# psy-ex/svt-av1-psy

Hardware: AMD Instinct MI355X
Metric: Mblocks/s per kernel (SAD, FwdTxfm2d, CDEF) + encoder fps @1080p preset 8 (higher is better)
Workload: dtype u8

## Files before the change

### svt-av1-psy_amd/csrc/sad.hip

```cpp
#include "svt_hip_common.h"
#include "../../include/svtav1_hip.h"
#include "hme_geom.h"
#include <vector>

namespace {

struct __attribute__((packed, aligned(4))) U64A4 { unsigned long long v; };
struct __attribute__((aligned(4))) u32x4_a4 { uint32_t x, y, z, w; };
struct __attribute__((aligned(16))) u32x4_a16 { uint32_t x, y, z, w; };

constexpr uint32_t MAX_SAD_VALUE = 128 * 128 * 255;
constexpr int      ME_TW         = 64;
constexpr int      ME_TH         = 32;
constexpr int      KEY_POS_BITS  = 11;
constexpr uint32_t ME_WAVE_MAX_W = 24, ME_WAVE_MAX_H = 16;

__device__ __forceinline__ void stage_rows_u8(uint32_t* lds, int pitch_dw, const uint8_t* g, uint32_t gstride, int width,
                                              int rows, int tid, int nthreads) {
    const int total = rows * pitch_dw;
    for (int i = tid; i < total; i += nthreads) {
        const int r   = i / pitch_dw;
        const int k   = i - r * pitch_dw;
        const int col = k * 4;
        uint32_t  v   = 0;
        if (col < width) {
            const uint8_t*  p    = g + (size_t)r * gstride + col;
            const uint32_t  sh   = (uint32_t)((uintptr_t)p & 3);
            const uint32_t* ap   = (const uint32_t*)(p - sh);
            const int       need = (width - col) < 4 ? (width - col) : 4;
            const uint32_t  lo   = ap[0];
            uint32_t        hi   = 0;
            if ((int)sh + need > 4) hi = ap[1];
            v = __builtin_amdgcn_alignbyte(hi, lo, sh);
            if (need < 4) v &= (1u << (8 * need)) - 1u;
        }
        lds[i] = v;
    }
}

struct __attribute__((packed, aligned(1))) u32x4_a1 { uint32_t x, y, z, w; };
struct __attribute__((packed, aligned(1))) u32_a1 { uint32_t x; };
struct __attribute__((aligned(8))) u32x2_a8 { uint32_t x, y; };

template <int NIT, int CL2>
__device__ __forceinline__ void stage_rows_load(uint32_t (&v)[NIT][4], const uint8_t* g, uint32_t gstride, int width, int rows, int tid) {
#pragma unroll
    for (int k = 0; k < NIT; ++k) {
        const int  idx = tid + 256 * k, r = idx >> CL2, col = (idx & ((1 << CL2) - 1)) * 16;
        const bool live = r < rows && col < width;
        const int  left = width - col;
        const int  back = (live && left < 16) ? 16 - left : 0;
        const uint8_t* p = g + (live ? (size_t)r * gstride + (size_t)(col - back) : (size_t)0);
        const u32x4_a1 t = *(const u32x4_a1*)p;
        v[k][0] = t.x; v[k][1] = t.y; v[k][2] = t.z; v[k][3] = t.w;
    }
#pragma unroll
    for (int k = 0; k < NIT; ++k) {
        const int  idx = tid + 256 * k, r = idx >> CL2, col = (idx & ((1 << CL2) - 1)) * 16;
        const bool live = r < rows && col < width;
        const int  left = width - col;
        uint32_t   x0 = live ? v[k][0] : 0u, x1 = live ? v[k][1] : 0u, x2 = live ? v[k][2] : 0u, x3 = live ? v[k][3] : 0u;
        if (live && left < 16) {
            const int back = 16 - left;
            if (back & 4) { x0 = x1; x1 = x2; x2 = x3; x3 = 0; }
            if (back & 8) { x0 = x2; x1 = x3; x2 = 0; x3 = 0; }
            const uint32_t bs = (uint32_t)back & 3u;
            x0 = __builtin_amdgcn_alignbyte(x1, x0, bs);
            x1 = __builtin_amdgcn_alignbyte(x2, x1, bs);
            x2 = __builtin_amdgcn_alignbyte(x3, x2, bs);
            x3 = __builtin_amdgcn_alignbyte(0u, x3, bs);
        }
        v[k][0] = x0; v[k][1] = x1; v[k][2] = x2; v[k][3] = x3;
    }
}
template <int NIT, int CL2>
__device__ __forceinline__ void stage_rows_store(const uint32_t (&v)[NIT][4], uint32_t* lds, int pitch_dw, int rows, int tid) {
#pragma unroll
    for (int k = 0; k < NIT; ++k) {
        const int idx = tid + 256 * k, r = idx >> CL2, c4 = (idx & ((1 << CL2) - 1)) * 4;
        if (r < rows) {
            uint32_t* o = lds + r * pitch_dw + c4;
            if (c4 + 0 < pitch_dw) *(u32x2_a8*)(o + 0) = u32x2_a8{v[k][0], v[k][1]};
            if (c4 + 2 < pitch_dw) *(u32x2_a8*)(o + 2) = u32x2_a8{v[k][2], v[k][3]};
        }
    }
}

template <int NT, int U>
__device__ __forceinline__ void stage_rows_wide_step(uint32_t* lds, const int pitch_dw, const uint8_t* g, const uint32_t gstride, const int width, const int total,
                                                     const int cpr, const int dr, const int dc, const int base, const int tid, int& r, int& c) {
    uint32_t v[U][4];
    int      rk[U], ck[U];
#pragma unroll
    for (int k = 0; k < U; ++k) {
        const int  idx = base + tid + NT * k, col = c * 16;
        rk[k] = r; ck[k] = c;
        const bool live = idx < total && col < width;
        const int  left = width - col;
        const int  back = (live && left < 16) ? 16 - left : 0;
        const uint8_t* p = g + (live ? (uint32_t)r * gstride + (uint32_t)(col - back) : 0u);
        const u32x4_a1 t = *(const u32x4_a1*)p;
        uint32_t x0 = live ? t.x : 0u, x1 = live ? t.y : 0u, x2 = live ? t.z : 0u, x3 = live ? t.w : 0u;
        if (back) {
            if (back & 4) { x0 = x1; x1 = x2; x2 = x3; x3 = 0; }
            if (back & 8) { x0 = x2; x1 = x3; x2 = 0; x3 = 0; }
            const uint32_t bs = (uint32_t)back & 3u;
            x0 = __builtin_amdgcn_alignbyte(x1, x0, bs);
            x1 = __builtin_amdgcn_alignbyte(x2, x1, bs);
            x2 = __builtin_amdgcn_alignbyte(x3, x2, bs);
            x3 = __builtin_amdgcn_alignbyte(0u, x3, bs);
        }
        v[k][0] = x0; v[k][1] = x1; v[k][2] = x2; v[k][3] = x3;
        r += dr; c += dc;
        if (c >= cpr) { c -= cpr; r++; }
    }
#pragma unroll
    for (int k = 0; k < U; ++k) {
        const int idx = base + tid + NT * k, c4 = ck[k] * 4;
        if (idx < total) {
            uint32_t* o = lds + rk[k] * pitch_dw + c4;
            if (c4 + 0 < pitch_dw) *(u32x2_a8*)(o + 0) = u32x2_a8{v[k][0], v[k][1]};
            if (c4 + 2 < pitch_dw) *(u32x2_a8*)(o + 2) = u32x2_a8{v[k][2], v[k][3]};
        }
    }
}
template <int NT = 256>
__device__ __forceinline__ void stage_rows_wide_any(uint32_t* lds, int pitch_dw, const uint8_t* g, uint32_t gstride, int width, int rows, int tid) {
    const int cpr = (pitch_dw + 3) >> 2, total = rows * cpr;
    const int dr = NT / cpr, dc = NT - dr * cpr;
    int       r = tid / cpr, c = tid - r * cpr;
    int base = 0;
    for (; total - base > 2 * NT; base += 4 * NT) stage_rows_wide_step<NT, 4>(lds, pitch_dw, g, gstride, width, total, cpr, dr, dc, base, tid, r, c);
    if (total - base > NT) stage_rows_wide_step<NT, 2>(lds, pitch_dw, g, gstride, width, total, cpr, dr, dc, base, tid, r, c);
    else if (total - base > 0) stage_rows_wide_step<NT, 1>(lds, pitch_dw, g, gstride, width, total, cpr, dr, dc, base, tid, r, c);
}

__device__ __forceinline__ uint32_t dpp_add_quad_xor1(uint32_t v) {
    return v + (uint32_t)__builtin_amdgcn_update_dpp(0, (int)v, 0xB1, 0xf, 0xf, false);
}
__device__ __forceinline__ uint32_t dpp_add_quad_xor2(uint32_t v) {
    return v + (uint32_t)__builtin_amdgcn_update_dpp(0, (int)v, 0x4E, 0xf, 0xf, false);
}
__device__ __forceinline__ uint32_t dpp_add_row_ror4(uint32_t v) {
    return v + (uint32_t)__builtin_amdgcn_update_dpp(0, (int)v, 0x124, 0xf, 0xf, false);
}
__device__ __forceinline__ uint32_t dpp_add_row_ror8(uint32_t v) {
    return v + (uint32_t)__builtin_amdgcn_update_dpp(0, (int)v, 0x128, 0xf, 0xf, false);
}
__device__ __forceinline__ uint32_t umin32(uint32_t a, uint32_t b) { return a < b ? a : b; }


constexpr int ME_PITCH = 34;

__device__ __forceinline__ uint32_t dpp_scatter_sum_quads(const uint32_t (&v)[4]) {
#ifdef SVT_HIP_EMU
    const uint32_t a0 = dpp_add_row_ror8(v[0]), a1 = dpp_add_row_ror8(v[1]), a2 = dpp_add_row_ror8(v[2]), a3 = dpp_add_row_ror8(v[3]);
    const uint32_t t0 = (uint32_t)__builtin_amdgcn_update_dpp((int)a0, (int)a2, 0xE4, 0xf, 0xc, false);
    const uint32_t t1 = (uint32_t)__builtin_amdgcn_update_dpp((int)a1, (int)a3, 0xE4, 0xf, 0xc, false);
    const uint32_t y  = (uint32_t)__builtin_amdgcn_update_dpp((int)t0, (int)t1, 0xE4, 0xf, 0xa, false);
    const uint32_t x  = y + (uint32_t)__builtin_amdgcn_update_dpp(0, (int)t0, 0x12C, 0xf, 0x5, false);
    return x + (uint32_t)__builtin_amdgcn_update_dpp(0, (int)t1, 0x124, 0xf, 0xa, false);
#else
    uint32_t t0, t1;
    asm("s_nop 1\n\t"
        "v_add_u32_dpp %0, %2, %2 row_ror:8 row_mask:0xf bank_mask:0x3\n\t"
        "v_add_u32_dpp %0, %4, %4 row_ror:8 row_mask:0xf bank_mask:0xc\n\t"
        "v_add_u32_dpp %1, %3, %3 row_ror:8 row_mask:0xf bank_mask:0x3\n\t"
        "v_add_u32_dpp %1, %5, %5 row_ror:8 row_mask:0xf bank_mask:0xc\n\t"
        "v_add_u32_dpp %0, %0, %0 row_ror:12 row_mask:0xf bank_mask:0x5\n\t"
        "s_nop 0\n\t"
        "v_add_u32_dpp %0, %1, %1 row_ror:4 row_mask:0xf bank_mask:0xa"
        : "=&v"(t0), "=&v"(t1)
        : "v"(v[0]), "v"(v[1]), "v"(v[2]), "v"(v[3]));
    return t0;
#endif
}

template <bool SUB, bool FULL, int PITCH = ME_PITCH>
__device__ __forceinline__ void me_search_strips(const uint32_t* __restrict__ win, const uint32_t (&s)[8][2], int Wt, int Ht, int g0, int gstep, int l,
                                                 uint32_t& best8, uint32_t& best16, uint32_t& best32, uint32_t& best64) {
    const int bx = (l & 1) | ((l >> 1) & 2) | ((l >> 2) & 4);
    const int by = ((l >> 1) & 1) | ((l >> 2) & 2) | ((l >> 3) & 4);
    const int q  = l & 3, c = (l >> 2) & 3;
    const int      G    = (Wt + 3) >> 2;
    const uint32_t qsel = 0x0c0c0100u + 0x0202u * (uint32_t)q;
    uint32_t       himask = 0xffff0000u;
    SVT_HIP_OPAQUE_I32(himask);
    constexpr uint32_t NO_STEP = 0x1ffffu;
    uint32_t       b16 = 0xffffffffu, b32 = 0xffffffffu, b64 = 0xffffffffu;
    for (int g = g0; g < G; g += gstep) {
        const uint32_t* colp   = win + (by * 8) * PITCH + bx * 2 + g;
        const int       nvalid = (Wt - 4 * g) < 4 ? (Wt - 4 * g) : 4;
        const uint32_t inv1 = nvalid > 1 ? 0u : 0xffffffffu, inv2 = nvalid > 2 ? 0u : 0xffffffffu, inv3 = nvalid > 3 ? 0u : 0xffffffffu;
        const uint32_t invq = q < nvalid ? 0u : 0xffffffffu;
        U64A4 ra[8], rb[8];
#pragma unroll
        for (int r = 0; r < 7; r++) {
            ra[r] = *(const U64A4*)(colp + r * PITCH);
            rb[r] = *(const U64A4*)(colp + r * PITCH + 1);
        }
        uint32_t pos = (uint32_t)(4 * g);
        for (int yb = 0; yb < Ht; yb += 8) {
            const uint32_t* rowp = colp + (yb + 7) * PITCH;
#pragma unroll
            for (int h = 0; h < 2; h++) {
                if (yb + 4 * h < Ht) {
                    uint32_t v[4] = {NO_STEP, NO_STEP, NO_STEP, NO_STEP};
#pragma unroll
                    for (int j = 0; j < 4; j++) {
                        const int i = 4 * h + j;
                        if (yb + i < Ht) {
                            ra[(i + 7) & 7] = *(const U64A4*)(rowp + i * PITCH);
                            rb[(i + 7) & 7] = *(const U64A4*)(rowp + i * PITCH + 1);
                            unsigned long long acc = 0;
#pragma unroll
                            for (int r = 0; r < 8; r += (SUB ? 2 : 1)) {
                                acc = __builtin_amdgcn_qsad_pk_u16_u8(ra[(i + r) & 7].v, s[r][0], acc);
                                acc = __builtin_amdgcn_qsad_pk_u16_u8(rb[(i + r) & 7].v, s[r][1], acc);
                            }
                            if (SUB) acc <<= 1;
                            const uint32_t lo = (uint32_t)acc, hi = (uint32_t)(acc >> 32);
                            const uint32_t p1 = FULL ? pos + 1 : ((pos + 1) | inv1), p2 = FULL ? pos + 2 : ((pos + 2) | inv2), p3 = FULL ? pos + 3 : ((pos + 3) | inv3);
                            const uint32_t k0 = (lo << 16) | pos, k1 = (lo & himask) | p1, k2 = (hi << 16) | p2, k3 = (hi & himask) | p3;
                            best8 = umin32(umin32(best8, k0), k1);
                            best8 = umin32(umin32(best8, k2), k3);
                            const uint32_t tlo = dpp_add_quad_xor2(dpp_add_quad_xor1(lo));
                            const uint32_t thi = dpp_add_quad_xor2(dpp_add_quad_xor1(hi));
                            v[j] = __builtin_amdgcn_perm(thi, tlo, qsel);
                            const uint32_t k16 = (v[j] << KEY_POS_BITS) | pos;
                            b16 = umin32(b16, FULL ? k16 : (k16 | invq));
                            pos += ME_TW;
                        }
                    }
                    const uint32_t gpos  = (uint32_t)(4 * g + ME_TW * (yb + 4 * h));
                    const uint32_t sad32 = dpp_scatter_sum_quads(v);
                    const uint32_t k32   = (sad32 << KEY_POS_BITS) | gpos;
                    b32 = umin32(b32, FULL ? k32 : (k32 | invq));
                    const auto     x16   = __builtin_amdgcn_permlane16_swap(sad32, sad32, false, false);
                    const uint32_t pair  = x16[0] + x16[1];
                    const auto     x32   = __builtin_amdgcn_permlane32_swap(pair, pair, false, false);
                    const uint32_t sad64 = x32[0] + x32[1];
                    const uint32_t k64   = (sad64 << KEY_POS_BITS) | gpos;
                    b64 = umin32(b64, FULL ? k64 : (k64 | invq));
                }
            }
        }
    }
    best16 = umin32(best16, b16 | (uint32_t)q);
    best32 = umin32(best32, b32 | (uint32_t)(q | (c << 6)));
    best64 = umin32(best64, b64 | (uint32_t)(q | (c << 6)));
}

template <bool SUB>
__global__ __launch_bounds__(256, 4) void me_fullpel_kernel(const uint8_t* __restrict__ src_base, const uint8_t* __restrict__ ref_base,
                                                         const SvtHipMeSearchDesc* __restrict__ descs, uint32_t n,
                                                         uint32_t tiles_x,
                                                         uint32_t* __restrict__ best_sad, uint32_t* __restrict__ best_mv,
                                                         unsigned long long* __restrict__ keys) {
    HIP_DYNAMIC_SHARED(uint32_t, smem)
    uint32_t* src_lds  = smem;
    uint32_t* best_lds = smem + 64 * 16;
    uint32_t* win      = smem + 64 * 16 + 88;

    const int      tid  = threadIdx.x;
    const uint32_t item = xcd_remap(blockIdx.x, n);
    const uint32_t tile = blockIdx.y;
    const SvtHipMeSearchDesc d = descs[item];
    const int W   = d.search_area_width, H = d.search_area_height;
    const int tx0 = (int)(tile % tiles_x) * ME_TW;
    const int ty0 = (int)(tile / tiles_x) * ME_TH;
    if (tx0 >= W || ty0 >= H) {
        if (tile == 0 && keys == nullptr && tid < SVT_HIP_ME_NUM_BLOCKS) {
            best_sad[(size_t)item * SVT_HIP_ME_NUM_BLOCKS + tid] = MAX_SAD_VALUE;
            best_mv[(size_t)item * SVT_HIP_ME_NUM_BLOCKS + tid]  = 0;
        }
        return;
    }
    const int Wt = (W - tx0) < ME_TW ? (W - tx0) : ME_TW;
    const int Ht = (H - ty0) < ME_TH ? (H - ty0) : ME_TH;

    {
        uint32_t vs[1][4], vw[3][4];
        stage_rows_load<1, 2>(vs, src_base + d.src_off, d.src_stride, 64, 64, tid);
        stage_rows_load<3, 3>(vw, ref_base + d.ref_off + (size_t)ty0 * d.ref_stride + tx0, d.ref_stride, 64 + Wt - 1, 64 + Ht - 1, tid);
        stage_rows_store<1, 2>(vs, src_lds, 16, 64, tid);
        stage_rows_store<3, 3>(vw, win, ME_PITCH, 64 + Ht - 1, tid);
    }
    if (tid < 88) best_lds[tid] = 0xffffffffu;
    __syncthreads();

    const int l  = tid & 63;
    const int wv = tid >> 6;
    uint32_t s[8][2];
    {
        const int bx = (l & 1) | ((l >> 1) & 2) | ((l >> 2) & 4);
        const int by = ((l >> 1) & 1) | ((l >> 2) & 2) | ((l >> 3) & 4);
#pragma unroll
        for (int r = 0; r < 8; r++) {
            s[r][0] = src_lds[(by * 8 + r) * 16 + bx * 2 + 0];
            s[r][1] = src_lds[(by * 8 + r) * 16 + bx * 2 + 1];
        }
    }
    uint32_t best8 = 0xffffffffu, best16 = 0xffffffffu, best32 = 0xffffffffu, best64 = 0xffffffffu;
    if ((Wt & 3) == 0) me_search_strips<SUB, true>(win, s, Wt, Ht, wv, 4, l, best8, best16, best32, best64);
    else me_search_strips<SUB, false>(win, s, Wt, Ht, wv, 4, l, best8, best16, best32, best64);

    atomicMin(&best_lds[21 + l], best8);
    atomicMin(&best_lds[5 + (l >> 2)], best16);
    atomicMin(&best_lds[1 + (l >> 4)], best32);
    atomicMin(&best_lds[0], best64);
    __syncthreads();
    if (tid < SVT_HIP_ME_NUM_BLOCKS) {
        const uint32_t key = best_lds[tid];
        const uint32_t sad = tid >= 21 ? (key >> 16) : (key >> KEY_POS_BITS);
        const int      X   = tx0 + (int)(key & 63u);
        const int      Y   = ty0 + (int)((key >> 6) & 31u);
        const size_t   o   = (size_t)item * SVT_HIP_ME_NUM_BLOCKS + tid;
        if (keys == nullptr) {
            best_sad[o] = sad;
            best_mv[o]  = ((uint32_t)(uint16_t)(Y + d.y_search_area_origin) << 16) | (uint16_t)(X + d.x_search_area_origin);
        } else {
            atomicMin(&keys[o], ((unsigned long long)sad << 32) | (unsigned long long)(uint32_t)(Y * W + X));
        }
    }
}

struct __attribute__((packed, aligned(1))) u32x2_a1 { uint32_t x, y; };
__device__ __forceinline__ uint32_t dpp_min_quad_xor1(uint32_t v) { return umin32(v, (uint32_t)__builtin_amdgcn_update_dpp(-1, (int)v, 0xB1, 0xf, 0xf, false)); }
__device__ __forceinline__ uint32_t dpp_min_quad_xor2(uint32_t v) { return umin32(v, (uint32_t)__builtin_amdgcn_update_dpp(-1, (int)v, 0x4E, 0xf, 0xf, false)); }
__device__ __forceinline__ uint32_t dpp_min_row_ror4(uint32_t v) { return umin32(v, (uint32_t)__builtin_amdgcn_update_dpp(-1, (int)v, 0x124, 0xf, 0xf, false)); }
__device__ __forceinline__ uint32_t dpp_min_row_ror8(uint32_t v) { return umin32(v, (uint32_t)__builtin_amdgcn_update_dpp(-1, (int)v, 0x128, 0xf, 0xf, false)); }

template <int NF, int PITCH>
__device__ __forceinline__ void stage_window_wave(uint32_t* lds, const uint8_t* g, const uint32_t gstride, const int width, const int rows, const int l) {
    constexpr int RPI = 64 / NF;
    const int     rem = width & 15, back = 16 - rem;
    const bool    p0 = rem != 0 && l < rows, p1 = rem != 0 && l + 64 < rows;
    u32x4_a1      t[2] = {{0u, 0u, 0u, 0u}, {0u, 0u, 0u, 0u}};
    const uint32_t tail_off = (uint32_t)l * gstride + (uint32_t)(width - 16);
    if (p0) t[0] = *(const u32x4_a1*)(g + tail_off);
    if (p1) t[1] = *(const u32x4_a1*)(g + (size_t)64 * gstride + tail_off);

    const int lr = l / NF, lc = l - lr * NF;
    if (lr < RPI) {
        const uint32_t goff = (uint32_t)lr * gstride + (uint32_t)lc * 16u;
        uint32_t*      lp   = lds + lr * PITCH + lc * 4;
        for (int r0 = 0; r0 < rows; r0 += 4 * RPI) {
            const uint8_t* gb = g + (size_t)r0 * gstride;
            u32x4_a1       v[4];
#pragma unroll
            for (int k = 0; k < 4; k++)
                if (r0 + k * RPI + lr < rows) v[k] = *(const u32x4_a1*)(gb + (size_t)(k * RPI) * gstride + goff);
#pragma unroll
            for (int k = 0; k < 4; k++)
                if (r0 + k * RPI + lr < rows) {
                    uint32_t* o = lp + (r0 + k * RPI) * PITCH;
                    *(u32x2_a8*)(o + 0) = u32x2_a8{v[k].x, v[k].y};
                    *(u32x2_a8*)(o + 2) = u32x2_a8{v[k].z, v[k].w};
                }
        }
    }
#pragma unroll
    for (int k = 0; k < 2; k++)
        if (k == 0 ? p0 : p1) {
            uint32_t x0 = t[k].x, x1 = t[k].y, x2 = t[k].z, x3 = t[k].w;
            if (back & 4) { x0 = x1; x1 = x2; x2 = x3; x3 = 0; }
            if (back & 8) { x0 = x2; x1 = x3; x2 = 0; x3 = 0; }
            const uint32_t bs = (uint32_t)back & 3u;
            x0 = __builtin_amdgcn_alignbyte(x1, x0, bs);
            x1 = __builtin_amdgcn_alignbyte(x2, x1, bs);
            x2 = __builtin_amdgcn_alignbyte(x3, x2, bs);
            x3 = __builtin_amdgcn_alignbyte(0u, x3, bs);
            uint32_t* o = lds + (l + 64 * k) * PITCH + NF * 4;
            if (NF * 4 + 0 < PITCH) *(u32x2_a8*)(o + 0) = u32x2_a8{x0, x1};
            if (NF * 4 + 2 < PITCH) *(u32x2_a8*)(o + 2) = u32x2_a8{x2, x3};
        }
}

template <bool SUB, int PITCH>
__global__ __launch_bounds__(256) void me_fullpel_wave_kernel(const uint8_t* __restrict__ src_base, const uint8_t* __restrict__ ref_base,
                                                              const SvtHipMeSearchDesc* __restrict__ descs, const uint32_t n, const int win_dw,
                                                              uint32_t* __restrict__ best_sad, uint32_t* __restrict__ best_mv) {
    HIP_DYNAMIC_SHARED(uint32_t, smem)
    const int      l    = threadIdx.x & 63, wv = __builtin_amdgcn_readfirstlane((int)(threadIdx.x >> 6));
    const uint32_t item = xcd_remap(blockIdx.x, gridDim.x) * 4 + (uint32_t)wv;
    if (item >= n) return;
    const SvtHipMeSearchDesc d = descs[item];
    const int    W = d.search_area_width, H = d.search_area_height;
    const size_t o = (size_t)item * SVT_HIP_ME_NUM_BLOCKS;
    if (W <= 0 || H <= 0) {
        for (int k = l; k < SVT_HIP_ME_NUM_BLOCKS; k += 64) { best_sad[o + k] = MAX_SAD_VALUE; best_mv[o + k] = 0; }
        return;
    }
    uint32_t* win = smem + wv * win_dw;
    const int bx = (l & 1) | ((l >> 1) & 2) | ((l >> 2) & 4);
    const int by = ((l >> 1) & 1) | ((l >> 2) & 2) | ((l >> 3) & 4);
    uint32_t  s[8][2];
    {
        const uint8_t* sp = src_base + d.src_off + (size_t)(by * 8) * d.src_stride + bx * 8;
#pragma unroll
        for (int r = 0; r < 8; r++) {
            const u32x2_a1 t = *(const u32x2_a1*)(sp + (size_t)r * d.src_stride);
            s[r][0] = t.x; s[r][1] = t.y;
        }
    }
    const int width = 64 + W - 1;
    if (PITCH >= 22 && (width >> 4) == 5) stage_window_wave<5, PITCH>(win, ref_base + d.ref_off, d.ref_stride, width, 64 + H - 1, l);
    else stage_window_wave<4, PITCH>(win, ref_base + d.ref_off, d.ref_stride, width, 64 + H - 1, l);
    __builtin_amdgcn_wave_barrier();

    uint32_t best8 = 0xffffffffu, best16 = 0xffffffffu, best32 = 0xffffffffu, best64 = 0xffffffffu;
    if ((W & 3) == 0) me_search_strips<SUB, true, PITCH>(win, s, W, H, 0, 1, l, best8, best16, best32, best64);
    else me_search_strips<SUB, false, PITCH>(win, s, W, H, 0, 1, l, best8, best16, best32, best64);
    best16 = dpp_min_quad_xor2(dpp_min_quad_xor1(best16));
    best32 = dpp_min_row_ror8(dpp_min_row_ror4(dpp_min_quad_xor2(dpp_min_quad_xor1(best32))));
    best64 = dpp_min_row_ror8(dpp_min_row_ror4(dpp_min_quad_xor2(dpp_min_quad_xor1(best64))));
    best64 = umin32(best64, (uint32_t)__shfl_xor((int)best64, 16));
    best64 = umin32(best64, (uint32_t)__shfl_xor((int)best64, 32));
    const int xo = d.x_search_area_origin, yo = d.y_search_area_origin;
    auto emit = [&](const int idx, const uint32_t key, const bool is8) {
        const uint32_t sad = is8 ? (key >> 16) : (key >> KEY_POS_BITS);
        const int      X = (int)(key & 63u), Y = (int)((key >> 6) & 31u);
        best_sad[o + idx] = sad;
        best_mv[o + idx]  = ((uint32_t)(uint16_t)(Y + yo) << 16) | (uint16_t)(X + xo);
    };
    emit(21 + l, best8, true);
    if ((l & 3) == 0) emit(5 + (l >> 2), best16, false);
    if ((l & 15) == 0) emit(1 + (l >> 4), best32, false);
    if (l == 0) emit(0, best64, false);
}

__global__ void me_finalize_kernel(const SvtHipMeSearchDesc* __restrict__ descs, uint32_t n, const unsigned long long* __restrict__ keys,
                                   uint32_t* __restrict__ best_sad, uint32_t* __restrict__ best_mv) {
    const uint32_t i = blockIdx.x * blockDim.x + threadIdx.x;
    if (i >= n * SVT_HIP_ME_NUM_BLOCKS) return;
    const SvtHipMeSearchDesc d   = descs[i / SVT_HIP_ME_NUM_BLOCKS];
    const unsigned long long key = keys[i];
    if (key == ~0ull) {
        best_sad[i] = MAX_SAD_VALUE;
        best_mv[i]  = 0;
        return;
    }
    const uint32_t pos = (uint32_t)key;
    const int      W   = d.search_area_width;
    const int      X = (int)(pos % (uint32_t)W), Y = (int)(pos / (uint32_t)W);
    best_sad[i]        = (uint32_t)(key >> 32);
    best_mv[i]         = ((uint32_t)(uint16_t)(Y + d.y_search_area_origin) << 16) | (uint16_t)(X + d.x_search_area_origin);
}

__device__ __forceinline__ uint32_t wave_sum(uint32_t v) {
    v += (uint32_t)__shfl_xor((int)v, 32);
    v += (uint32_t)__shfl_xor((int)v, 16);
    v = dpp_add_row_ror8(v);
    v = dpp_add_row_ror4(v);
    v = dpp_add_quad_xor2(v);
    v = dpp_add_quad_xor1(v);
    return v;
}

template <int CHUNK>
__device__ __forceinline__ uint32_t sad_chunks(const uint8_t* __restrict__ src, const uint8_t* __restrict__ ref, uint32_t ss, uint32_t rs,
                                               int cpr, int cshift, int total, int l) {
    uint32_t sad = 0;
    for (int i0 = l; i0 < total; i0 += 256) {
        uint32_t av[4][CHUNK / 4], bv[4][CHUNK / 4];
#pragma unroll
        for (int k = 0; k < 4; ++k) {
            const int  i  = i0 + 64 * k;
            const bool in = i < total;
            const int  r  = cshift >= 0 ? (i >> cshift) : (i / cpr);
            const int  c  = i - r * cpr;
            const uint8_t* pa = src + (size_t)r * ss + c * CHUNK;
            const uint8_t* pb = ref + (size_t)r * rs + c * CHUNK;
            if (CHUNK == 16) {
                u32x4_a1 a = {0, 0, 0, 0}, b = {0, 0, 0, 0};
                if (in) { a = *(const u32x4_a1*)pa; b = *(const u32x4_a1*)pb; }
                av[k][0] = a.x; av[k][CHUNK / 4 > 1 ? 1 : 0] = a.y; av[k][CHUNK / 4 > 2 ? 2 : 0] = a.z; av[k][CHUNK / 4 > 3 ? 3 : 0] = a.w;
                bv[k][0] = b.x; bv[k][CHUNK / 4 > 1 ? 1 : 0] = b.y; bv[k][CHUNK / 4 > 2 ? 2 : 0] = b.z; bv[k][CHUNK / 4 > 3 ? 3 : 0] = b.w;
            } else {
                u32_a1 a = {0}, b = {0};
                if (in) { a = *(const u32_a1*)pa; b = *(const u32_a1*)pb; }
                av[k][0] = a.x; bv[k][0] = b.x;
            }
        }
#pragma unroll
        for (int k = 0; k < 4; ++k)
#pragma unroll
            for (int j = 0; j < CHUNK / 4; ++j) sad = __builtin_amdgcn_sad_u8(av[k][j], bv[k][j], sad);
    }
    return sad;
}

__global__ __launch_bounds__(256) void sad_nxm_kernel(const uint8_t* __restrict__ src_base, const uint8_t* __restrict__ ref_base,
                                                      const SvtHipSadPair* __restrict__ pairs, uint32_t n, int width, int height,
                                                      uint32_t* __restrict__ sad_out) {
    const int      l    = threadIdx.x & 63;
    const uint32_t pair = xcd_remap(blockIdx.x, gridDim.x) * 4 + (threadIdx.x >> 6);
    if (pair >= n) return;
    const SvtHipSadPair p   = pairs[pair];
    const uint8_t*      src = src_base + p.src_off;
    const uint8_t*      ref = ref_base + p.ref_off;
    uint32_t            sad = 0;
    if ((width & 15) == 0) {
        const int cpr = width >> 4;
        sad = sad_chunks<16>(src, ref, p.src_stride, p.ref_stride, cpr, (cpr & (cpr - 1)) ? -1 : __builtin_ctz(cpr), cpr * height, l);
    } else if ((width & 3) == 0) {
        const int cpr = width >> 2;
        sad = sad_chunks<4>(src, ref, p.src_stride, p.ref_stride, cpr, (cpr & (cpr - 1)) ? -1 : __builtin_ctz(cpr), cpr * height, l);
    } else {
        const int total = width * height;
        for (int i = l; i < total; i += 64) {
            const int r = i / width, c = i - r * width;
            const int a = src[(size_t)r * p.src_stride + c], b = ref[(size_t)r * p.ref_stride + c];
            sad += (uint32_t)(a > b ? a - b : b - a);
        }
    }
    sad = wave_sum(sad);
    if (l == 0) sad_out[pair] = sad;
}

constexpr int SADP_PPW = 4;
struct SadRegs { uint32_t a[4][4], b[4][4]; };
__device__ __forceinline__ void sadp_issue(SadRegs& r, const uint8_t* __restrict__ src, const uint8_t* __restrict__ ref, const SvtHipSadPair& p, const int cpr,
                                           const int cshift, const int total, const int l) {
#pragma unroll
    for (int k = 0; k < 4; ++k) {
        const int  i  = l + 64 * k;
        const bool in = i < total;
        const int  rr = i >> cshift, c = i - (rr << cshift);
        u32x4_a1 a = {0, 0, 0, 0}, b = {0, 0, 0, 0};
        if (in) {
            a = *(const u32x4_a1*)(src + p.src_off + (size_t)rr * p.src_stride + c * 16);
            b = *(const u32x4_a1*)(ref + p.ref_off + (size_t)rr * p.ref_stride + c * 16);
        }
        r.a[k][0] = a.x; r.a[k][1] = a.y; r.a[k][2] = a.z; r.a[k][3] = a.w;
        r.b[k][0] = b.x; r.b[k][1] = b.y; r.b[k][2] = b.z; r.b[k][3] = b.w;
    }
}
__device__ __forceinline__ uint32_t sadp_reduce(const SadRegs& r) {
    uint32_t sad = 0;
#pragma unroll
    for (int k = 0; k < 4; ++k)
#pragma unroll
        for (int j = 0; j < 4; ++j) sad = __builtin_amdgcn_sad_u8(r.a[k][j], r.b[k][j], sad);
    return wave_sum(sad);
}
__global__ __launch_bounds__(256) void sad_nxm_pipe_kernel(const uint8_t* __restrict__ src_base, const uint8_t* __restrict__ ref_base,
                                                           const SvtHipSadPair* __restrict__ pairs, uint32_t n, int cshift , int total,
                                                           uint32_t* __restrict__ sad_out) {
    const int      l     = threadIdx.x & 63, w = __builtin_amdgcn_readfirstlane(threadIdx.x >> 6);
    const uint32_t first = xcd_remap(blockIdx.x, gridDim.x) * (4 * SADP_PPW) + (uint32_t)w;
    if (first >= n) return;
    const int cpr = 1 << cshift;
    SadRegs   cur, nxt;
    sadp_issue(cur, src_base, ref_base, pairs[first], cpr, cshift, total, l);
#pragma unroll
    for (int k = 0; k < SADP_PPW; ++k) {
        const uint32_t pair = first + 4u * (uint32_t)k, np = pair + 4u;
        const bool     more = k + 1 < SADP_PPW && np < n;
        if (more) sadp_issue(nxt, src_base, ref_base, pairs[np], cpr, cshift, total, l);
        const uint32_t sad = sadp_reduce(cur);
        if (l == 0) sad_out[pair] = sad;
        if (!more) break;
        cur = nxt;
    }
}

constexpr int SADS_SPW = 4;
struct StripRegs { uint32_t a[4][4], b[4][4]; };
__device__ __forceinline__ void strip_issue(StripRegs& r, const uint8_t* __restrict__ sp, const uint8_t* __restrict__ rp, const uint32_t ss, const uint32_t rs,
                                            const int row0, const int ro, const int height, const bool live) {
#pragma unroll
    for (int k = 0; k < 4; ++k) {
        const int row = row0 + 4 * k;
        u32x4_a1  a = {0, 0, 0, 0}, b = {0, 0, 0, 0};
        if (live && row + ro < height) {
            a = *(const u32x4_a1*)(sp + (size_t)row * ss);
            b = *(const u32x4_a1*)(rp + (size_t)row * rs);
        }
        r.a[k][0] = a.x; r.a[k][1] = a.y; r.a[k][2] = a.z; r.a[k][3] = a.w;
        r.b[k][0] = b.x; r.b[k][1] = b.y; r.b[k][2] = b.z; r.b[k][3] = b.w;
    }
}
__device__ __forceinline__ uint32_t strip_consume(const StripRegs& r, uint32_t sad) {
#pragma unroll
    for (int k = 0; k < 4; ++k)
#pragma unroll
        for (int j = 0; j < 4; ++j) sad = __builtin_amdgcn_sad_u8(r.a[k][j], r.b[k][j], sad);
    return sad;
}
__global__ __launch_bounds__(256) void sad_nxm_strip_kernel(const uint8_t* __restrict__ src_base, const uint8_t* __restrict__ ref_base,
                                                            const SvtHipSadPair* __restrict__ pairs, const uint32_t n, const int cshift ,
                                                            const int height, uint32_t* __restrict__ sad_out) {
    const int      l = threadIdx.x & 63, w = __builtin_amdgcn_readfirstlane(threadIdx.x >> 6);
    const int      cpr = 1 << cshift, nb = 16 >> cshift;
    const int      sb = (l & 15) >> cshift, j = l & (cpr - 1), ro = l >> 4;
    const int      groups = (height + 15) >> 4;
    const uint32_t strip0 = (xcd_remap(blockIdx.x, gridDim.x) * 4 + (uint32_t)w) * SADS_SPW;
    if (strip0 * (uint32_t)nb >= n) return;
    const uint8_t *sp = nullptr, *rp = nullptr;
    uint32_t       ss = 0, rs = 0;
    bool           live = false;
    auto open_strip = [&](const int k) {
        const uint32_t pair = (strip0 + (uint32_t)k) * (uint32_t)nb + (uint32_t)sb;
        live = k < SADS_SPW && pair < n;
        if (live) {
            const SvtHipSadPair p = pairs[pair];
            sp = src_base + p.src_off + (size_t)ro * p.src_stride + j * 16;
            rp = ref_base + p.ref_off + (size_t)ro * p.ref_stride + j * 16;
            ss = p.src_stride; rs = p.ref_stride;
        }
    };
    StripRegs cur, nxt;
    open_strip(0);
    strip_issue(cur, sp, rp, ss, rs, 0, ro, height, live);
    for (int k = 0; k < SADS_SPW; ++k) {
        if ((strip0 + (uint32_t)k) * (uint32_t)nb >= n) break;
        const bool     mine = live;
        uint32_t       sad  = 0;
        const uint32_t out  = (strip0 + (uint32_t)k) * (uint32_t)nb + (uint32_t)sb;
        for (int g = 0; g < groups; ++g) {
            if (g + 1 < groups) {
                strip_issue(nxt, sp, rp, ss, rs, 16 * (g + 1), ro, height, live);
            } else {
                open_strip(k + 1);
                strip_issue(nxt, sp, rp, ss, rs, 0, ro, height, live);
            }
            sad = strip_consume(cur, sad);
            cur = nxt;
        }
        for (int m = 1; m < cpr; m <<= 1) sad += (uint32_t)__shfl_xor((int)sad, m);
        sad += (uint32_t)__shfl_xor((int)sad, 16);
        sad += (uint32_t)__shfl_xor((int)sad, 32);
        if (mine && j == 0 && ro == 0) sad_out[out] = sad;
    }
}

__global__ __launch_bounds__(64) void sad_16b_kernel(const uint16_t* __restrict__ src, uint32_t src_stride, const uint16_t* __restrict__ ref,
                                                     uint32_t ref_stride, int width, int height, uint32_t* __restrict__ out) {
    const int l     = threadIdx.x;
    uint32_t  sad   = 0;
    const int total = width * height;
    for (int i = l; i < total; i += 64) {
        const int r = i / width, c = i - r * width;
        const int a = src[(size_t)r * src_stride + c], b = ref[(size_t)r * ref_stride + c];
        sad += (uint32_t)(a > b ? a - b : b - a);
    }
    sad = wave_sum(sad);
    if (l == 0) out[0] = sad;
}

template <int LXG>
__device__ __forceinline__ void sad_loop_item(uint32_t* smem, unsigned long long& wg_best, const uint8_t* __restrict__ src_base,
                                              const uint8_t* __restrict__ ref_base, const SvtHipSadLoopDesc& d, const uint32_t item, const uint32_t tile,
                                              const uint32_t tiles_x, unsigned long long* __restrict__ keys) {
    constexpr int TW = 4 << LXG, TH = 256 >> LXG;
    const int tid = threadIdx.x;
    const int W = d.search_area_width, H = d.search_area_height;
    const int bw = d.block_width, bh = d.block_height;
    const int tx0 = (int)(tile % tiles_x) * TW, ty0 = (int)(tile / tiles_x) * TH;
    if (tx0 >= W || ty0 >= H) return;
    const int Wt = (W - tx0) < TW ? (W - tx0) : TW;
    const int Ht = (H - ty0) < TH ? (H - ty0) : TH;
    const int src_pitch = ((bw + 15) >> 4) << 2;
    const int win_w     = bw + Wt - 1;
    const int win_pitch = (((bw + TW + 3) >> 2) + 3) & ~1;
    uint32_t* src_lds   = smem;
    uint32_t* win       = smem + src_pitch * bh;
    stage_rows_u8(src_lds, src_pitch, src_base + d.src_off, d.src_stride, bw, bh, tid, 256);
    if (tid == 0) wg_best = ~0ull;
    const int rstep    = (int)(d.ref_stride / d.src_stride_raw);
    const int win_rows = Ht + rstep * (bh - 1);
    const uint8_t* wsrc = ref_base + d.ref_off + (size_t)ty0 * d.src_stride_raw + tx0;
    if (win_w >= 16) stage_rows_wide_any(win, win_pitch, wsrc, d.src_stride_raw, win_w, win_rows, tid);
    else stage_rows_u8(win, win_pitch, wsrc, d.src_stride_raw, win_w, win_rows, tid, 256);
    __syncthreads();

    const int gx = tid & ((1 << LXG) - 1), yy = tid >> LXG;
    const bool skip_rule = (bw == 16) && (bh <= 16) && d.skip_search_line;
    unsigned long long best = ~0ull;
    if (yy < Ht && 4 * gx < Wt && !(skip_rule && (((ty0 + yy) & 1) == 0))) {
        uint32_t sad[4] = {0, 0, 0, 0};
        const int full_dw = bw >> 2, tail = bw & 3;
        for (int y = 0; y < bh; y++) {
            const uint32_t* rrow = win + (yy + rstep * y) * win_pitch + gx;
            const uint32_t* srow = src_lds + y * src_pitch;
            unsigned long long acc = 0;
            uint32_t prev = rrow[0];
            int      k    = 0;
            for (; k + 4 <= full_dw; k += 4) {
                const u32x4_a16 sv = *(const u32x4_a16*)(srow + k);
                const U64A4     n0 = *(const U64A4*)(rrow + k + 1), n1 = *(const U64A4*)(rrow + k + 3);
                const uint32_t  r1 = (uint32_t)n0.v, r2 = (uint32_t)(n0.v >> 32), r3 = (uint32_t)n1.v, r4 = (uint32_t)(n1.v >> 32);
                acc  = __builtin_amdgcn_qsad_pk_u16_u8(((unsigned long long)r1 << 32) | prev, sv.x, acc);
                acc  = __builtin_amdgcn_qsad_pk_u16_u8(n0.v, sv.y, acc);
                acc  = __builtin_amdgcn_qsad_pk_u16_u8(((unsigned long long)r3 << 32) | r2, sv.z, acc);
                acc  = __builtin_amdgcn_qsad_pk_u16_u8(n1.v, sv.w, acc);
                prev = r4;
                if ((k & 12) == 12) {
                    sad[0] += (uint32_t)acc & 0xffffu; sad[1] += (uint32_t)(acc >> 16) & 0xffffu;
                    sad[2] += (uint32_t)(acc >> 32) & 0xffffu; sad[3] += (uint32_t)(acc >> 48);
                    acc = 0;
                }
            }
            for (; k < full_dw; k++) {
                const uint32_t next = rrow[k + 1];
                acc  = __builtin_amdgcn_qsad_pk_u16_u8(((unsigned long long)next << 32) | prev, srow[k], acc);
                prev = next;
            }
            sad[0] += (uint32_t)acc & 0xffffu; sad[1] += (uint32_t)(acc >> 16) & 0xffffu;
            sad[2] += (uint32_t)(acc >> 32) & 0xffffu; sad[3] += (uint32_t)(acc >> 48);
            if (tail) {
                const uint32_t mask = (1u << (8 * tail)) - 1u;
                const uint32_t next = rrow[full_dw + 1];
                const uint32_t sv   = srow[full_dw] & mask;
#pragma unroll
                for (int j = 0; j < 4; j++) {
                    const uint32_t rv = __builtin_amdgcn_alignbyte(next, prev, (uint32_t)j) & mask;
                    sad[j]            = __builtin_amdgcn_sad_u8(rv, sv, sad[j]);
                }
            }
        }
#pragma unroll
        for (int j = 0; j < 4; j++) {
            const int X = tx0 + 4 * gx + j;
            if (4 * gx + j < Wt) {
                const unsigned long long key = ((unsigned long long)sad[j] << 32) | (uint32_t)((ty0 + yy) * W + X);
                best = key < best ? key : best;
            }
        }
    }
    atomicMin(&wg_best, best);
// ... 963 lines not shown
```

Before: 26640.

## Batch tail-row 32/64 SAD reductions across strips and coalesce key emits

In the ME full-pel search, the 32x32/64x64 cross-lane reductions are skipped for a trailing single-row half-step when the search height leaves one row. Those tail rows are instead accumulated per column group and reduced once every four strips. The final 64-wide min uses permlane swaps in place of shuffles, and the 21 block-level results are gathered with one ds_bpermute so 21 lanes emit in parallel instead of through divergent branches. This cuts cross-lane ops in the inner loop but adds bookkeeping, and the new position encoding risks correctness errors.

Result: faster. 26930, median of 6 (+1.1%).

```diff
diff --git a/svt-av1-psy_amd/csrc/sad.hip b/svt-av1-psy_amd/csrc/sad.hip
--- a/svt-av1-psy_amd/csrc/sad.hip
+++ b/svt-av1-psy_amd/csrc/sad.hip
@@ -188,6 +188,9 @@
     SVT_HIP_OPAQUE_I32(himask);
     constexpr uint32_t NO_STEP = 0x1ffffu;
     uint32_t       b16 = 0xffffffffu, b32 = 0xffffffffu, b64 = 0xffffffffu;
+    constexpr uint32_t NO_SUM = 0x7ffffu;
+    uint32_t       p32 = NO_SUM, b32p = 0xffffffffu, b64p = 0xffffffffu;
+    int            kc = 0;
     for (int g = g0; g < G; g += gstep) {
         const uint32_t* colp   = win + (by * 8) * PITCH + bx * 2 + g;
         const int       nvalid = (Wt - 4 * g) < 4 ? (Wt - 4 * g) : 4;
@@ -200,6 +203,7 @@
             rb[r] = *(const U64A4*)(colp + r * PITCH + 1);
         }
         uint32_t pos = (uint32_t)(4 * g);
+        uint32_t v0  = 0;
         for (int yb = 0; yb < Ht; yb += 8) {
             const uint32_t* rowp = colp + (yb + 7) * PITCH;
 #pragma unroll
@@ -232,23 +236,43 @@
                             pos += ME_TW;
                         }
                     }
-                    const uint32_t gpos  = (uint32_t)(4 * g + ME_TW * (yb + 4 * h));
-                    const uint32_t sad32 = dpp_scatter_sum_quads(v);
-                    const uint32_t k32   = (sad32 << KEY_POS_BITS) | gpos;
-                    b32 = umin32(b32, FULL ? k32 : (k32 | invq));
-                    const auto     x16   = __builtin_amdgcn_permlane16_swap(sad32, sad32, false, false);
-                    const uint32_t pair  = x16[0] + x16[1];
-                    const auto     x32   = __builtin_amdgcn_permlane32_swap(pair, pair, false, false);
-                    const uint32_t sad64 = x32[0] + x32[1];
-                    const uint32_t k64   = (sad64 << KEY_POS_BITS) | gpos;
-                    b64 = umin32(b64, FULL ? k64 : (k64 | invq));
+                    v0 = v[0];
+                    if (yb + 4 * h + 1 < Ht) {
+                        const uint32_t gpos  = (uint32_t)(4 * g + ME_TW * (yb + 4 * h));
+                        const uint32_t sad32 = dpp_scatter_sum_quads(v);
+                        const uint32_t k32   = (sad32 << KEY_POS_BITS) | gpos;
+                        b32 = umin32(b32, FULL ? k32 : (k32 | invq));
+                        const auto     x16   = __builtin_amdgcn_permlane16_swap(sad32, sad32, false, false);
+                        const uint32_t pair  = x16[0] + x16[1];
+                        const auto     x32   = __builtin_amdgcn_permlane32_swap(pair, pair, false, false);
+                        const uint32_t sad64 = x32[0] + x32[1];
+                        const uint32_t k64   = (sad64 << KEY_POS_BITS) | gpos;
+                        b64 = umin32(b64, FULL ? k64 : (k64 | invq));
+                    }
                 }
+            }
+        }
+        if ((Ht & 3) == 1) {
+            const uint32_t sum = dpp_add_row_ror4(dpp_add_row_ror8(v0));
+            if (c == kc && (FULL || q < nvalid)) p32 = sum;
+            if (++kc == 4 || g + gstep >= G) {
+                const uint32_t gpos  = (uint32_t)(4 * (g - (kc - 1) * gstep) + ME_TW * (Ht - 1));
+                b32p = umin32(b32p, (p32 << KEY_POS_BITS) | gpos);
+                const auto     x16   = __builtin_amdgcn_permlane16_swap(p32, p32, false, false);
+                const uint32_t pair  = x16[0] + x16[1];
+                const auto     x32   = __builtin_amdgcn_permlane32_swap(pair, pair, false, false);
+                const uint32_t sad64 = x32[0] + x32[1];
+                b64p = umin32(b64p, (sad64 << KEY_POS_BITS) | gpos);
+                p32 = NO_SUM;
+                kc  = 0;
             }
         }
     }
     best16 = umin32(best16, b16 | (uint32_t)q);
     best32 = umin32(best32, b32 | (uint32_t)(q | (c << 6)));
     best64 = umin32(best64, b64 | (uint32_t)(q | (c << 6)));
+    best32 = umin32(best32, b32p | (uint32_t)(q | (4 * gstep * c)));
+    best64 = umin32(best64, b64p | (uint32_t)(q | (4 * gstep * c)));
 }
 
 template <bool SUB>
@@ -415,8 +439,12 @@
     best16 = dpp_min_quad_xor2(dpp_min_quad_xor1(best16));
     best32 = dpp_min_row_ror8(dpp_min_row_ror4(dpp_min_quad_xor2(dpp_min_quad_xor1(best32))));
     best64 = dpp_min_row_ror8(dpp_min_row_ror4(dpp_min_quad_xor2(dpp_min_quad_xor1(best64))));
-    best64 = umin32(best64, (uint32_t)__shfl_xor((int)best64, 16));
-    best64 = umin32(best64, (uint32_t)__shfl_xor((int)best64, 32));
+    {
+        const auto x16 = __builtin_amdgcn_permlane16_swap(best64, best64, false, false);
+        best64         = umin32(x16[0], x16[1]);
+        const auto x32 = __builtin_amdgcn_permlane32_swap(best64, best64, false, false);
+        best64         = umin32(x32[0], x32[1]);
+    }
     const int xo = d.x_search_area_origin, yo = d.y_search_area_origin;
     auto emit = [&](const int idx, const uint32_t key, const bool is8) {
         const uint32_t sad = is8 ? (key >> 16) : (key >> KEY_POS_BITS);
@@ -425,9 +453,11 @@
         best_mv[o + idx]  = ((uint32_t)(uint16_t)(Y + yo) << 16) | (uint16_t)(X + xo);
     };
     emit(21 + l, best8, true);
-    if ((l & 3) == 0) emit(5 + (l >> 2), best16, false);
-    if ((l & 15) == 0) emit(1 + (l >> 4), best32, false);
-    if (l == 0) emit(0, best64, false);
+    const int      q    = l & 3;
+    const uint32_t mine = q == 1 ? best16 : (q == 2 ? best32 : best64);
+    const int      r32  = 64 * l - 56, r16 = 16 * l - 76;
+    const uint32_t key  = (uint32_t)__builtin_amdgcn_ds_bpermute(l < 5 ? (r32 > 0 ? r32 : 0) : r16, (int)mine);
+    if (l < 21) emit(l, key, false);
 }
 
 __global__ void me_finalize_kernel(const SvtHipMeSearchDesc* __restrict__ descs, uint32_t n, const unsigned long long* __restrict__ keys,
```
